# hassony2/handobjectconsist

Hardware: AMD Instinct MI355X
Metric: trainmeshwarp iters/sec (render+warp, B=64, 256x256) (higher is better)
Workload: dtype f32; 1 GPU; trainmeshwarp.py consist step, per-GPU B=64, 256x256, hand 778v/1552f + object 1002v/2000f (7104 faces after fill-back), ResNet-18 fp32 (MIOpen convolutions, channels-last, + fused HIP BatchNorm/ReLU/residual/max-pool kernels), Adam; global_batch=64, image_size=256, parallelism=dp1

## Files before the change

handobjectconsist_amd/_lib.py:

```python
import ctypes
import os

import torch

_HERE = os.path.dirname(os.path.abspath(__file__))
LIB_PATH = os.environ.get("HOC_LIB_PATH") or os.path.join(_HERE, "libmeshraster_hip.so")
ABI_VERSION = 9
FLAG_REFERENCE_ALGO = 1
FLAG_SPARSE_TILES = 2
FLAG_OUTPUT_ZEROED = 4
FLAG_TILE_PER_WORKGROUP = 8
FLAG_TILE_LIST_CLEARED = 16
FLAG_FORCE_PARTS = 1 << 24
FLAG_ONE_WORKGROUP_PER_IMAGE = 32 << 24
FLAG_PARTS_IN_ONE_LAUNCH = 64 << 24
FLAG_PLAIN_DIVISIONS = 4096 << 8
FLAG_FORCE_GATHER = 32 << 8
FLAG_COUNT_PIXEL_MAP_TERMS = 1024 << 8
CRITERION_L1 = 0
CRITERION_L2 = 1
DTYPE_F32, DTYPE_BF16, DTYPE_U8 = 0, 1, 2
DTYPE_CODES = {torch.float32: DTYPE_F32, torch.bfloat16: DTYPE_BF16, torch.uint8: DTYPE_U8}
IMAGE_DTYPES = (torch.float32, torch.bfloat16)
MASK_DTYPES = (torch.float32, torch.uint8)
# ... 88 lines not shown
    "mr_pair_step_forward": (_I, [_P, _P]),
    "mr_pair_step_backward": (_I, [_P, _P]),
    "mr_frames_to_batch_workspace_bytes": (_L, [_I, _I, _I]),
    "mr_frames_to_batch": (_I, [_P] * 3 + [_F] * 6 + [_P, _L, _P, _P] + [_I] * 6 + [_P]),
    "mr_frames_to_batch_typed": (_I, [_P] * 3 + [_F] * 6 + [_P, _L, _P, _P] + [_I] * 6 + [_P, _I, _I]),
    "mr_frames_color_augment_workspace_bytes": (_L, [_I, _I, _I]),
    "mr_frames_color_augment": (_I, [_P] * 7 + [_L, _I, _I, _I, _P]),
    "mr_jpeg_info": (_I, [_P, _L, _P]),
    "mr_jpeg_packed_bytes": (_L, [_I] * 5),
    "mr_jpeg_entropy_decode": (_I, [_P, _L, _P, _L]),
    "mr_jpeg_reconstruct_workspace_bytes": (_L, [_I] * 6),
    "mr_jpeg_reconstruct": (_I, [_P] + [_I] * 6 + [_P, _P, _L, _P]),
    "mr_png_packed_bytes": (_L, [_I] * 3),
    "mr_png_unfilter_workspace_bytes": (_L, [_I] * 4),
    "mr_png_unfilter": (_I, [_P] + [_I] * 4 + [_P, _P, _P]),
    "mr_frames_resize_taps": (_I, [_I, _I]),
    "mr_frames_resize_tables": (_I, [_I, _I, _P, _P]),
    "mr_frames_resize_plan": (_I, [_I] * 4 + [_P]),
    "mr_frames_resize_workspace_bytes": (_I, [_I] * 5),
    "mr_frames_resize": (_I, [_P, _I, _I, _I, _P, _I, _I] + [_P] * 6),
    "mr_bn_act_forward": (_I, [_P] * 6 + [_F, _I, _I, _I, _P, _I, _I, _I, _P]),
    "mr_bn_act_backward_workspace_bytes": (_L, [_I, _I]),
    "mr_bn_act_backward": (_I, [_P] * 8 + [_F, _I, _I, _I] + [_P] * 5 + [_L, _I, _I, _I, _P]),
    "mr_bn_add_bn_act_forward": (_I, [_P] * 6 + [_F] + [_P] * 4 + [_F, _I, _P, _I, _I, _I, _P]),
    "mr_bn_add_bn_act_backward_workspace_bytes": (_L, [_I, _I]),
    "mr_bn_add_bn_act_backward": (_I, [_P] * 8 + [_F] + [_P] * 4 + [_F, _I] + [_P] * 7 + [_L, _I, _I, _I, _P]),
    "mr_stem_pool_forward": (_I, [_P] * 5 + [_F, _I, _I, _P, _P, _I, _I, _I, _I, _P]),
    "mr_stem_pool_records_bytes": (_L, [_I, _I, _I, _I]),
    "mr_stem_pool_backward_workspace_bytes": (_L, [_I, _I, _I, _I]),
    "mr_stem_pool_backward": (_I, [_P] * 8 + [_F, _I, _I] + [_P] * 4 + [_L, _I, _I, _I, _I, _P]),
    "mr_stem_pool_param_grads": (_I, [_P] * 7 + [_F, _I] + [_P] * 3 + [_L, _I, _I, _I, _I, _P]),
    "mr_stem_conv_wrw_tiling": (_I, [_P] * 3),
    "mr_stem_conv_wrw_workspace_bytes": (_L, [_I, _I, _I, _I]),
    "mr_stem_conv_wrw": (_I, [_P] * 7 + [_F, _P, _P, _I, _P, _L] + [_I] * 8 + [_P]),
}

_lib = None


def load():
    global _lib
    if _lib is not None:
        return _lib
    if not os.path.exists(LIB_PATH):
        raise RuntimeError(
            f"{LIB_PATH} is missing: the HIP extension has not been built. Run "
# ... 95 lines not shown
```

handobjectconsist_amd/csrc/bn_device.hpp:

```cpp
#pragma once
#include <initializer_list>

#include "mr_common.hpp"

namespace mr {

__device__ __forceinline__ float act_to_f32(float v) { return v; }
__device__ __forceinline__ float act_to_f32(bf16_t v) { return bf16_to_f32(v); }
template <typename T> __device__ __forceinline__ T act_from_f32(float v);
template <> __device__ __forceinline__ float act_from_f32<float>(float v) { return v; }
template <> __device__ __forceinline__ bf16_t act_from_f32<bf16_t>(float v) { return f32_to_bf16(v); }

template <typename T> struct Vec4;
template <> struct Vec4<float> { typedef float4 type; };
template <> struct Vec4<bf16_t> { typedef ushort4 type; };

template <typename T>
__device__ __forceinline__ float load1(const void* base, int64_t o) { return act_to_f32(static_cast<const T*>(base)[o]); }
template <typename T>
__device__ __forceinline__ void store1(void* base, int64_t o, float v) { static_cast<T*>(base)[o] = act_from_f32<T>(v); }
template <typename T>
__device__ __forceinline__ void load4(const void* base, int64_t o, float* v) {
    const typename Vec4<T>::type t = *reinterpret_cast<const typename Vec4<T>::type*>(static_cast<const T*>(base) + o);
    v[0] = act_to_f32(t.x); v[1] = act_to_f32(t.y); v[2] = act_to_f32(t.z); v[3] = act_to_f32(t.w);
}
template <typename T>
__device__ __forceinline__ void store4(void* base, int64_t o, const float* v) {
    typename Vec4<T>::type t;
    t.x = act_from_f32<T>(v[0]); t.y = act_from_f32<T>(v[1]); t.z = act_from_f32<T>(v[2]); t.w = act_from_f32<T>(v[3]);
    *reinterpret_cast<typename Vec4<T>::type*>(static_cast<T*>(base) + o) = t;
}

template <typename T>
__device__ __forceinline__ float load1_grad(const void* grad_y, const void* grad_y2, int64_t o) {
    float g = load1<T>(grad_y, o);
    if (grad_y2) g += load1<T>(grad_y2, o);
    return g;
}
template <typename T>
__device__ __forceinline__ void load4_grad(const void* grad_y, const void* grad_y2, int64_t o, float* g) {
    load4<T>(grad_y, o, g);
    if (grad_y2) {
        float g2[4];
        load4<T>(grad_y2, o, g2);
#pragma unroll
        for (int i = 0; i < 4; i++) g[i] += g2[i];
    }
}

__device__ __forceinline__ float relu_nan(float z) { return z > 0.0f ? z : (z != z ? z : 0.0f); }

struct BnAffine {
    const float* weight;
// ... 144 lines not shown
```

handobjectconsist_amd/csrc/frozen_bn.hip:

```cpp
#include "bn_device.hpp"

namespace mr {

struct BnParams {
    const void* x;
    const void* residual;
    BnAffine bn;
    int relu;
    int N, C, HW, split;
    void* y;
    const void* grad_y;
    const void* grad_y2;
    void* grad_x;
    void* grad_residual;
    float* partial;
};

template <bool BACKWARD>
__device__ __forceinline__ void bn_act_element(float x, bool has_res, float res, float grad, bool relu, float mean, float a,
                                               float b, float& out, float& gres, float& sum_g, float& sum_gd) {
    const float d = x - mean;
    float z = d * a + b;
    if (has_res) z = z + res;
    if (!BACKWARD) {
        out = relu ? relu_nan(z) : z;
    } else {
        const float g = (relu && !(z > 0.0f)) ? 0.0f : grad;
        gres = g;
        out = g * a;
        sum_g += g;
        sum_gd += g * d;
    }
}

template <typename T, bool VEC, bool BACKWARD>
__global__ __launch_bounds__(256) void bn_act_kernel(BnParams p) {
    const int c = blockIdx.x / p.split, k = blockIdx.x % p.split;
    const int n0 = (int)((int64_t)k * p.N / p.split), n1 = (int)((int64_t)(k + 1) * p.N / p.split);
// ... 21 lines not shown
#pragma unroll
        for (int i = 0; i < W; i++) bn_act_element<BACKWARD>(xv[i], has_res, rv[i], gv[i], relu, mean, a, b, out[i], gres[i], s[0], s[1]);
        void* dst = BACKWARD ? p.grad_x : p.y;
        if (VEC) {
            store4<T>(dst, o, out);
            if (BACKWARD && p.grad_residual) store4<T>(p.grad_residual, o, gres);
        } else {
            store1<T>(dst, o, out[0]);
            if (BACKWARD && p.grad_residual) store1<T>(p.grad_residual, o, gres[0]);
        }
    }
    if (BACKWARD && p.partial) {
        float t[2];
        wave_block_sums<2>(s, t);
        if (threadIdx.x == 0) {
            p.partial[(int64_t)c * p.split + k] = t[0];
            p.partial[(int64_t)(p.C + c) * p.split + k] = t[1];
        }
    }
}

constexpr int BN_NHWC_BLOCKS = 2048;

template <typename T, bool BACKWARD>
__global__ __launch_bounds__(256) void bn_act_nhwc_kernel(BnParams p) {
    const NhwcLane l = nhwc_lane(p.bn, p.C);
    const int64_t pixels = (int64_t)p.N * p.HW;
    const bool relu = p.relu != 0, has_res = p.residual != nullptr;
    float s[2][4] = {};
    for (int64_t px = l.first(); px < pixels; px += l.stride()) {
        const int64_t o = px * p.C + l.c0;
        float xv[4], rv[4] = {}, gv[4] = {}, out[4], gres[4];
        load4<T>(p.x, o, xv);
        if (has_res) load4<T>(p.residual, o, rv);
        if (BACKWARD) load4_grad<T>(p.grad_y, p.grad_y2, o, gv);
#pragma unroll
        for (int i = 0; i < 4; i++)
            bn_act_element<BACKWARD>(xv[i], has_res, rv[i], gv[i], relu, l.mean[i], l.a[i], l.b[i], out[i], gres[i], s[0][i], s[1][i]);
        store4<T>(BACKWARD ? p.grad_x : p.y, o, out);
        if (BACKWARD && p.grad_residual) store4<T>(p.grad_residual, o, gres);
    }
    if (BACKWARD && p.partial) nhwc_block_sums<2>(l, s, p.partial, p.C);
}

struct BnAddParams {
    const void* x;
    const void* xd;
    BnAffine bn, bn_d;
    int N, C, HW;
    void* y;
    const void* grad_y;
    const void* grad_y2;
    void* grad_x;
    void* grad_xd;
    float* partial;
};

template <typename T, bool BACKWARD>
__global__ __launch_bounds__(256) void bn_add_bn_act_nhwc_kernel(BnAddParams p) {
    const NhwcLane l = nhwc_lane(p.bn, p.C), ld = nhwc_lane(p.bn_d, p.C);
    const int64_t pixels = (int64_t)p.N * p.HW;
    float s[3][4] = {};
    for (int64_t px = l.first(); px < pixels; px += l.stride()) {
// ... 102 lines not shown
    if (channels_last && channels > 0 && !nhwc_channels_ok(channels)) return MR_ERR_BADARG;
    if (channels == 0) return MR_OK;
    if (!weight || !bias || !running_mean || !running_var) return MR_ERR_BADARG;
    const bool want_params = grad_weight || grad_bias;
    if (batch_size == 0 || plane == 0) return zero_param_grads({grad_weight, grad_bias}, channels, (hipStream_t)stream);
    if (!grad_y || !x || !grad_x) return MR_ERR_BADARG;
    if (grad_residual && !residual) return MR_ERR_BADARG;
    if (want_params && (!workspace || workspace_bytes < mr_bn_act_backward_workspace_bytes(batch_size, channels)))
        return MR_ERR_BADARG;
    BnParams p = bn_fill(x, residual, weight, bias, running_mean, running_var, eps, relu, batch_size, channels, plane);
    p.grad_y = grad_y; p.grad_y2 = grad_y2; p.grad_x = grad_x; p.grad_residual = grad_residual;
    p.partial = want_params ? static_cast<float*>(workspace) : nullptr;
    if (!bn_sizes_ok(p)) return MR_ERR_BADARG;
    const bool all_aligned = aligned4(x, act_dtype) && aligned4(grad_y, act_dtype) && aligned4(grad_y2, act_dtype) &&
                             aligned4(grad_x, act_dtype) && aligned4(residual, act_dtype) && aligned4(grad_residual, act_dtype);
    if (channels_last && !all_aligned) return MR_ERR_BADARG;
    const int64_t slots = bn_act_slots(batch_size, channels, channels_last, (int64_t)batch_size * plane);
    bn_launch<true>(p, act_dtype, channels_last, plane % 4 == 0 && all_aligned, (int)slots, (hipStream_t)stream);
    MR_CHECK_LAUNCH();
    if (!want_params) return MR_OK;
    return launch_bn_finish<2>(p.partial, slots, channels, bn_finish_out(running_var, eps, grad_weight, grad_bias), (hipStream_t)stream);
}

namespace mr {
static BnAddParams bn_add_fill(const void* x, const void* xd, const BnAffine& bn, const BnAffine& bn_d, int N, int C, int plane) {
    BnAddParams p{};
    p.x = x; p.xd = xd; p.bn = bn; p.bn_d = bn_d; p.N = N; p.C = C; p.HW = plane;
    return p;
}
template <bool BACKWARD>
static void bn_add_launch(const BnAddParams& p, int act_dtype, int blocks, hipStream_t s) {
    dispatch_act(act_dtype, [&](auto tag) {
        using T = typename decltype(tag)::type;
        hipLaunchKernelGGL((bn_add_bn_act_nhwc_kernel<T, BACKWARD>), dim3((unsigned)blocks), dim3(256), 0, s, p);
    });
}
}

extern "C" int mr_bn_add_bn_act_forward(const void* x, const void* xd, const float* weight, const float* bias,
                                        const float* running_mean, const float* running_var, float eps,
                                        const float* weight_d, const float* bias_d, const float* running_mean_d,
                                        const float* running_var_d, float eps_d, int act_dtype, void* y, int batch_size,
                                        int channels, int plane, mr_stream_t stream) {
    using namespace mr;
    if (batch_size < 0 || channels < 0 || plane < 0 || (act_dtype != 0 && act_dtype != 1)) return MR_ERR_BADARG;
    if (channels > 0 && !nhwc_channels_ok(channels)) return MR_ERR_BADARG;
// ... 54 lines not shown
```

handobjectconsist_amd/csrc/stem_pool.hip:

```cpp
#include "bn_device.hpp"

namespace mr {

struct StemParams {
    const void* x;
    BnAffine bn;
    int N, C, H, W, OH, OW;
    int tiles_x, tiles_y;
    void* y;
    const void* grad_y;
    const void* grad_y2;
    void* grad_x;
    float* partial;
    unsigned char* argmax;
};

constexpr int SP_TX = 32, SP_TY = 16;
constexpr int SP_IH = 2 * SP_TY + 3, SP_IW = 2 * SP_TX + 8, SP_C0 = 4;
constexpr int SP_LDW = SP_IW + 1;

template <typename T, bool KEEP_D>
__device__ __forceinline__ void load_tile(const StemParams& p, const T* xp, int oy0, int ox0, float mean, float a,
                                          float b, float (*zt)[SP_LDW], float (*dt)[SP_LDW]) {
    const int iy0 = 2 * oy0 - 1, ix0 = 2 * ox0 - SP_C0;
// ... 199 lines not shown
                g[0] += id.x == code ? gv[0] : 0.0f;
                g[1] += id.y == code ? gv[1] : 0.0f;
                g[2] += id.z == code ? gv[2] : 0.0f;
                g[3] += id.w == code ? gv[3] : 0.0f;
            }
        }
#pragma unroll
        for (int i = 0; i < 4; i++) {
            const float d = xv[i] - l.mean[i];
            const float gm = (d * l.a[i] + l.b[i] > 0.0f) ? g[i] : 0.0f;
            out[i] = gm * l.a[i];
            s[0][i] += gm;
            s[1][i] += gm * d;
        }
        store4<T>(p.grad_x, ip * p.C + l.c0, out);
    }
    if (p.partial) nhwc_block_sums<2>(l, s, p.partial, p.C);
}

__device__ __forceinline__ unsigned char* sp_rec_codes(const StemParams& p) {
    return p.argmax + (int64_t)p.N * p.OH * p.OW * p.C * 4;
}

template <typename T>
__global__ __launch_bounds__(256) void stem_pool_rec_forward_kernel(StemParams p) {
    const NhwcLane l = nhwc_lane(p.bn, p.C);
    float* rec_d = reinterpret_cast<float*>(p.argmax);
    unsigned char* rec_code = sp_rec_codes(p);
    const int QH = (p.OH + 1) >> 1, QW = (p.OW + 1) >> 1;
    const int64_t total = (int64_t)p.N * QH * QW;
    for (int64_t q = l.first(); q < total; q += l.stride()) {
        const int qx = (int)(q % QW), qy = (int)((q / QW) % QH), n = (int)(q / ((int64_t)QW * QH));
        const int oy0 = 2 * qy, ox0 = 2 * qx;
        float best[2][2][4], bd[2][2][4];
        unsigned bi[2][2][4];
#pragma unroll
        for (int w = 0; w < 4; w++)
#pragma unroll
            for (int i = 0; i < 4; i++) { best[w >> 1][w & 1][i] = -__builtin_inff(); bd[w >> 1][w & 1][i] = 0.0f; bi[w >> 1][w & 1][i] = 0; }
#pragma unroll
        for (int r = 0; r < 5; r++) {
            const int iy = 2 * oy0 - 1 + r;
            if (iy < 0 || iy >= p.H) continue;
#pragma unroll
            for (int c = 0; c < 5; c++) {
                const int ix = 2 * ox0 - 1 + c;
                if (ix < 0 || ix >= p.W) continue;
                float xv[4];
                load4<T>(p.x, (((int64_t)n * p.H + iy) * p.W + ix) * p.C + l.c0, xv);
#pragma unroll
                for (int i = 0; i < 4; i++) {
                    const float d = xv[i] - l.mean[i];
                    const float v = relu_nan(d * l.a[i] + l.b[i]);
#pragma unroll
                    for (int wy = 0; wy < 2; wy++) {
                        const int kh = r - 2 * wy;
                        if (kh < 0 || kh > 2) continue;
#pragma unroll
                        for (int wx = 0; wx < 2; wx++) {
                            const int kw = c - 2 * wx;
                            if (kw < 0 || kw > 2) continue;
                            if (v > best[wy][wx][i] || v != v) { best[wy][wx][i] = v; bd[wy][wx][i] = d; bi[wy][wx][i] = (unsigned)(kh * 3 + kw); }
                        }
                    }
                }
            }
        }
#pragma unroll
        for (int wy = 0; wy < 2; wy++)
#pragma unroll
            for (int wx = 0; wx < 2; wx++) {
                const int oy = oy0 + wy, ox = ox0 + wx;
                if (oy >= p.OH || ox >= p.OW) continue;
                const int64_t o = (((int64_t)n * p.OH + oy) * p.OW + ox) * p.C + l.c0;
                store4<T>(p.y, o, best[wy][wx]);
                *reinterpret_cast<float4*>(rec_d + o) = make_float4(bd[wy][wx][0], bd[wy][wx][1], bd[wy][wx][2], bd[wy][wx][3]);
                *reinterpret_cast<uchar4*>(rec_code + o) = make_uchar4((unsigned char)bi[wy][wx][0], (unsigned char)bi[wy][wx][1],
                                                                       (unsigned char)bi[wy][wx][2], (unsigned char)bi[wy][wx][3]);
            }
    }
}

template <typename T>
__global__ __launch_bounds__(256) void stem_pool_rec_backward_kernel(StemParams p) {
    const NhwcLane l = nhwc_lane(p.bn, p.C);
    const float* rec_d = reinterpret_cast<const float*>(p.argmax);
    const unsigned char* rec_code = sp_rec_codes(p);
    const int QH = (p.H >> 1) + 1, QW = (p.W >> 1) + 1;
    const int64_t total = (int64_t)p.N * QH * QW;
    float sums[2][4] = {};
// ... 237 lines not shown
```

handobjectconsist_amd/csrc/stem_wrw.hip:

```cpp
#include "bn_device.hpp"

namespace mr {

constexpr int SW_TY = 4, SW_TX = 32;
constexpr int SW_BLOCKS = 512;
constexpr int SW_C = 64;
constexpr int SW_TAPS = 7 * 7 * 3;
constexpr int SW_NB = 5;
constexpr int SW_OUT = SW_C * SW_TAPS;
constexpr int SW_PH = 2 * SW_TY + 5;
constexpr int SW_PROW = (2 * SW_TX + 5) * 3;
constexpr int SW_PW = 213;
constexpr int SW_G = SW_TY * SW_TX * SW_C;
constexpr int SW_LDS = SW_G + SW_PH * SW_PW;
constexpr int SW_FIN_RUNS = 8, SW_FIN_RUN = SW_BLOCKS / SW_FIN_RUNS;
static_assert(SW_LDS >= SW_C * SW_NB * 32, "the wave reduction reuses the tile's LDS");
static_assert(SW_OUT % 32 == 0, "finish kernel: 32 outputs per workgroup");

typedef float f32x16 __attribute__((ext_vector_type(16)));

struct WrwParams {
    const float* grad_y;
    const float* grad_y2;
    const float* rec_d;
    const unsigned char* rec_code;
    BnAffine bn;
    const float* image;
    float* partial;
    int N, Hin, Win, H, W, OH, OW;
    int tiles_x, tiles_y;
    int64_t tiles;
};

__device__ __forceinline__ void wrw_keep(float& v) { asm volatile("" : "+v"(v)); }
__device__ __forceinline__ void wrw_keep(unsigned& v) { asm volatile("" : "+v"(v)); }
__device__ __forceinline__ void wrw_keep(float4& v) { asm volatile("" : "+v"(v.x), "+v"(v.y), "+v"(v.z), "+v"(v.w)); }

__global__ __launch_bounds__(256, 2) void stem_conv_wrw_kernel(WrwParams p) {
    __shared__ __attribute__((aligned(16))) float lds[SW_LDS];
    float* const G = lds;
    float* const patch = lds + SW_G;
    const int tid = threadIdx.x, lane = tid & 63, wave = tid >> 6, half = lane >> 5, l31 = lane & 31;

    const int c0 = 4 * (tid & 15), qcol = tid >> 4;
    float a[4], b[4];
#pragma unroll
    for (int i = 0; i < 4; i++) {
        float mean;
        channel_consts(p.bn, c0 + i, mean, a[i], b[i]);
    }

    const float* aptr[2];
    const float* bptr[SW_NB];
#pragma unroll
    for (int m = 0; m < 2; m++) aptr[m] = G + (wave * SW_TX + 16 * half) * SW_C + ((l31 + 32 * m) ^ (32 * half));
#pragma unroll
    for (int n = 0; n < SW_NB; n++) {
        const int t = l31 + 32 * n;
        const int off = t < SW_TAPS ? (t / 21) * SW_PW + t % 21 : 0;
        bptr[n] = patch + 2 * wave * SW_PW + 6 * 16 * half + off;
// ... 4 lines not shown
    for (int m = 0; m < 2; m++)
#pragma unroll
        for (int n = 0; n < SW_NB; n++)
#pragma unroll
            for (int r = 0; r < 16; r++) acc[m][n][r] = 0.0f;

    const int per_image = p.tiles_x * p.tiles_y;
    for (int64_t tile = blockIdx.x; tile < p.tiles; tile += gridDim.x) {
        const int n = (int)(tile / per_image), rem = (int)(tile - (int64_t)n * per_image);
        const int cy0 = (rem / p.tiles_x) * SW_TY, cx0 = (rem % p.tiles_x) * SW_TX;

        {
            const int iy0 = 2 * cy0 - 3, ix0 = 2 * cx0 - 3;
            const int c = tid < SW_PROW ? tid : SW_PROW - 1, ix = ix0 + c / 3;
            const bool col = ix >= 0 && ix < p.Win;
            const float* src = p.image + (int64_t)n * p.Hin * p.Win * 3 + (col ? ix0 * 3 + c : 0);
            float pv[SW_PH];
#pragma unroll
            for (int r = 0; r < SW_PH; r++) {
                const int iy = iy0 + r, iyc = iy < 0 ? 0 : (iy >= p.Hin ? p.Hin - 1 : iy);
                pv[r] = src[(int64_t)iyc * p.Win * 3];
            }
#pragma unroll
            for (int r = 0; r < SW_PH; r++) wrw_keep(pv[r]);
#pragma unroll
            for (int r = 0; r < SW_PH; r++) {
                const int iy = iy0 + r;
                if (!col || iy < 0 || iy >= p.Hin) pv[r] = 0.0f;
            }
            if (tid < SW_PROW) {
#pragma unroll
                for (int r = 0; r < SW_PH; r++) patch[r * SW_PW + tid] = pv[r];
            }
        }

#pragma unroll 1
        for (int qr = 0; qr < SW_TY / 2; qr++) {
            float s[2][2][4];
            unsigned code[2][2][4];
            unsigned idw[2][2];
            float4 dv[2][2], g1[2][2], g2[2][2];
#pragma unroll
            for (int j = 0; j < 2; j++)
#pragma unroll
                for (int k = 0; k < 2; k++) {
                    const int wy = (cy0 >> 1) + qr + j, wx = (cx0 >> 1) + qcol + k;
                    const int64_t o = (((int64_t)n * p.OH + (wy < p.OH ? wy : p.OH - 1)) * p.OW + (wx < p.OW ? wx : p.OW - 1)) * SW_C + c0;
                    idw[j][k] = *reinterpret_cast<const unsigned*>(p.rec_code + o);
                    dv[j][k] = *reinterpret_cast<const float4*>(p.rec_d + o);
                    g1[j][k] = *reinterpret_cast<const float4*>(p.grad_y + o);
                    g2[j][k] = *reinterpret_cast<const float4*>((p.grad_y2 ? p.grad_y2 : p.grad_y) + o);
                }
#pragma unroll
            for (int j = 0; j < 2; j++)
#pragma unroll
                for (int k = 0; k < 2; k++) { wrw_keep(idw[j][k]); wrw_keep(dv[j][k]); wrw_keep(g1[j][k]); wrw_keep(g2[j][k]); }
#pragma unroll
            for (int j = 0; j < 2; j++)
#pragma unroll
                for (int k = 0; k < 2; k++) {
                    const int wy = (cy0 >> 1) + qr + j, wx = (cx0 >> 1) + qcol + k;
                    const bool win = wy < p.OH && wx < p.OW;
                    const float d[4] = {dv[j][k].x, dv[j][k].y, dv[j][k].z, dv[j][k].w};
                    const float gv[4] = {p.grad_y2 ? g1[j][k].x + g2[j][k].x : g1[j][k].x, p.grad_y2 ? g1[j][k].y + g2[j][k].y : g1[j][k].y,
                                         p.grad_y2 ? g1[j][k].z + g2[j][k].z : g1[j][k].z, p.grad_y2 ? g1[j][k].w + g2[j][k].w : g1[j][k].w};
#pragma unroll
                    for (int i = 0; i < 4; i++) {
                        code[j][k][i] = win ? (idw[j][k] >> (8 * i)) & 255u : 255u;
                        s[j][k][i] = (d[i] * a[i] + b[i] > 0.0f) ? gv[i] : 0.0f;
                    }
                }
#pragma unroll
            for (int pr = 0; pr < 2; pr++)
#pragma unroll
                for (int pc = 0; pc < 2; pc++) {
                    const int py = 2 * qr + pr, px = 2 * qcol + pc;
                    float g[4] = {0.0f, 0.0f, 0.0f, 0.0f};
#pragma unroll
                    for (int dy = 0; dy < 2; dy++) {
// ... 135 lines not shown
```

handobjectconsist_amd/models/synthnet.py:

```python
import os

import numpy as np
import torch
import torch.nn.functional as F
from torch import nn

from handobjectconsist_amd import _lib
from handobjectconsist_amd.models import manoadapt
from handobjectconsist_amd.nn import frozen_bn
from handobjectconsist_amd.utils import project as camproject
from handobjectconsist_amd.utils import synth


USE_HIP_BN = os.environ.get("HOC_HIP_BN", "1") == "1"


USE_CHANNELS_LAST = os.environ.get("HOC_CHANNELS_LAST", "1") == "1"


USE_STEM_WRW = True


def _fused_bn(bn, x):
    if not (USE_HIP_BN and not bn.training and x.is_cuda):
        return False
    out_dtype = torch.get_autocast_dtype("cuda") if torch.is_autocast_enabled("cuda") else x.dtype
    return out_dtype in (torch.float32, torch.bfloat16)


class BasicBlock(nn.Module):
    expansion = 1

    def __init__(self, inplanes, planes, stride=1, downsample=None):
        super().__init__()
        self.conv1 = nn.Conv2d(inplanes, planes, 3, stride, 1, bias=False)
        self.bn1 = nn.BatchNorm2d(planes)
        self.relu = nn.ReLU(inplace=True)
        self.conv2 = nn.Conv2d(planes, planes, 3, 1, 1, bias=False)
        self.bn2 = nn.BatchNorm2d(planes)
        self.downsample = downsample

    def forward_fused(self, x, x_identity, dup=False):
        if self.downsample is not None:
            xd = self.downsample[0](x_identity)
            out = frozen_bn.bn_act(self.conv1(x), self.bn1)
            return frozen_bn.bn_add_bn_act(self.conv2(out), self.bn2, xd, self.downsample[1], dup=dup)
        out = frozen_bn.bn_act(self.conv1(x), self.bn1)
        return frozen_bn.bn_act(self.conv2(out), self.bn2, residual=x_identity, dup=dup)

    def forward(self, x):
        if _fused_bn(self.bn1, x):
            return self.forward_fused(x, x)
        residual = x if self.downsample is None else self.downsample(x)
        out = self.relu(self.bn1(self.conv1(x)))
        out = self.bn2(self.conv2(out))
        return self.relu(out + residual)


class ResNet18Features(nn.Module):

    def __init__(self):
        super().__init__()
        self.inplanes = 64
        self.conv1 = nn.Conv2d(3, 64, kernel_size=7, stride=2, padding=3, bias=False)
        self.bn1 = nn.BatchNorm2d(64)
        self.relu = nn.ReLU(inplace=True)
        self.maxpool = nn.MaxPool2d(kernel_size=3, stride=2, padding=1)
        self.layer1 = self._make_layer(64, 2)
        self.layer2 = self._make_layer(128, 2, stride=2)
        self.layer3 = self._make_layer(256, 2, stride=2)
        self.layer4 = self._make_layer(512, 2, stride=2)
# ... 486 lines not shown
```

handobjectconsist_amd/nn/frozen_bn.py:

```python
import torch
import torch.nn.functional as F

from handobjectconsist_amd import _lib


_ACT_DTYPES = {torch.float32: 0, torch.bfloat16: 1}


def _nhwc_channels_ok(C):
    return 4 <= C <= 1024 and 1024 % C == 0


def _layout(x):
    if (x.dim() == 4 and _nhwc_channels_ok(x.shape[1]) and not x.is_contiguous()
            and x.is_contiguous(memory_format=torch.channels_last)):
        return x, 1
    return x.contiguous(), 0


def _aligned(t, cl):
    if t is not None and cl and t.data_ptr() % (4 * t.element_size()):
        return t.clone(memory_format=torch.preserve_format)
    return t

# ... 47 lines not shown
        return (y, y.view_as(y)) if dup else y

    @staticmethod
    def backward(ctx, grad_y, grad_y2=None):
        xc, rc, w, b, m, v = ctx.saved_tensors
        eps, relu, N, C, plane, cl = ctx.cfg
        need_x, need_r, need_w, need_b = ctx.needs_input_grad[:4]
        g, g2 = _incoming(grad_y, grad_y2, xc.dtype, cl)
        if g is None:
            return (None,) * 9
        dev = xc.device
        grad_x = torch.empty_like(xc)
        grad_r = torch.empty_like(xc) if (rc is not None and need_r) else None
        grad_w = torch.empty_like(w) if need_w else None
        grad_b = torch.empty_like(b) if need_b else None
        work, wbytes = _workspace("mr_bn_act_backward_workspace_bytes", (N, C), dev, need_w or need_b)
        _lib.call("mr_bn_act_backward", _lib.ptr(g), _lib.ptr(g2), _lib.ptr(xc), _lib.ptr(rc), _lib.ptr(w), _lib.ptr(b), _lib.ptr(m),
                  _lib.ptr(v), eps, int(relu), _ACT_DTYPES[xc.dtype], cl, _lib.ptr(grad_x), _lib.ptr(grad_r), _lib.ptr(grad_w),
                  _lib.ptr(grad_b),
                  _lib.ptr(work), wbytes, N, C, plane, _lib.stream_ptr(dev))
        return (grad_x if need_x else None), grad_r, grad_w, grad_b, None, None, None, None, None


def bn_act(x, bn, residual=None, relu=True, dup=False):
    if bn.training or not bn.track_running_stats:
        raise RuntimeError("bn_act needs frozen BatchNorm statistics (module.eval())")
    return _BnActFunction.apply(x, residual, bn.weight, bn.bias, bn.running_mean, bn.running_var, bn.eps, relu, dup)


class _BnAddBnActFunction(torch.autograd.Function):

    @staticmethod
    def forward(ctx, x, xd, weight, bias, running_mean, running_var, eps, weight_d, bias_d, running_mean_d,
                running_var_d, eps_d, dup):
        ctx.set_materialize_grads(False)
        _lib.check_cuda(x, xd, weight, bias, running_mean, running_var, weight_d, bias_d, running_mean_d, running_var_d)
        xc, xdc = _aligned(x, 1), _aligned(xd, 1)
        N, C = xc.shape[:2]
        plane = xc[0, 0].numel() if N and C else 0
        chan = _channel_arrays(C, weight, bias, running_mean, running_var, weight_d, bias_d, running_mean_d, running_var_d)
        y = torch.empty_like(xc)
        _lib.call("mr_bn_add_bn_act_forward", _lib.ptr(xc), _lib.ptr(xdc), *[_lib.ptr(t) for t in chan[:4]], float(eps),
                  *[_lib.ptr(t) for t in chan[4:]], float(eps_d), _ACT_DTYPES[xc.dtype], _lib.ptr(y), N, C, plane,
                  _lib.stream_ptr(xc.device))
        ctx.save_for_backward(xc, xdc, *chan)
        ctx.cfg = (float(eps), float(eps_d), N, C, plane)
        return (y, y.view_as(y)) if dup else y

    @staticmethod
# ... 153 lines not shown
```

include/meshraster_hip.h:

```cpp
#ifndef MESHRASTER_HIP_H
#define MESHRASTER_HIP_H

#include <stdint.h>

#ifdef __cplusplus
extern "C" {
#endif

#define MR_OK 0
#define MR_ERR_BADARG (-1)
#define MR_ERR_NOTIMPL (-2)

#define MR_FLAG_REFERENCE_ALGO 1
#define MR_FLAG_SPARSE_TILES 2
#define MR_FLAG_OUTPUT_ZEROED 4
#define MR_FLAG_TILE_PER_WORKGROUP 8
#define MR_FLAG_TILE_LIST_CLEARED 16
#define MR_FLAG_FORCE_PARTS (1 << 24)
#define MR_FLAG_ONE_WORKGROUP_PER_IMAGE (32 << 24)
#define MR_FLAG_PARTS_IN_ONE_LAUNCH (64 << 24)
#define MR_FLAG_PLAIN_DIVISIONS (4096 << 8)
#define MR_FLAG_FORCE_GATHER (32 << 8)
#define MR_FLAG_COUNT_PIXEL_MAP_TERMS (1024 << 8)

// ... 532 lines not shown
#define MR_RESIZE_MAX_TAPS 33
#define MR_RESIZE_PLAN_INTS 8
MR_API int mr_frames_resize_taps(int in_size, int out_size);
MR_API int mr_frames_resize_tables(int in_size, int out_size, int* bounds, int* coeffs);
MR_API int mr_frames_resize_plan(int src_w, int src_h, int dst_w, int dst_h, int* plan);
MR_API int mr_frames_resize_workspace_bytes(int num_frames, int src_w, int src_h, int dst_w, int dst_h);
MR_API int mr_frames_resize(const unsigned char* frames_in, int num_frames, int src_w, int src_h,
                            unsigned char* frames_out, int dst_w, int dst_h, const int* bounds_x, const int* coeffs_x,
                            const int* bounds_y, const int* coeffs_y, void* workspace, mr_stream_t stream);

MR_API int mr_bn_act_forward(const void* x, const void* residual, const float* weight, const float* bias,
                             const float* running_mean, const float* running_var, float eps, int relu,
                             int act_dtype, int channels_last, void* y, int batch_size, int channels,
                             int plane, mr_stream_t stream);
MR_API int64_t mr_bn_act_backward_workspace_bytes(int batch_size, int channels);
MR_API int mr_bn_act_backward(const void* grad_y, const void* grad_y2, const void* x, const void* residual,
                              const float* weight, const float* bias, const float* running_mean,
                              const float* running_var, float eps, int relu, int act_dtype,
                              int channels_last, void* grad_x, void* grad_residual, float* grad_weight,
                              float* grad_bias,
                              void* workspace, int64_t workspace_bytes, int batch_size, int channels,
                              int plane, mr_stream_t stream);

MR_API int mr_bn_add_bn_act_forward(const void* x, const void* xd, const float* weight, const float* bias,
                                    const float* running_mean, const float* running_var, float eps,
                                    const float* weight_d, const float* bias_d, const float* running_mean_d,
                                    const float* running_var_d, float eps_d, int act_dtype, void* y,
                                    int batch_size, int channels, int plane, mr_stream_t stream);
MR_API int64_t mr_bn_add_bn_act_backward_workspace_bytes(int batch_size, int channels);
MR_API int mr_bn_add_bn_act_backward(const void* grad_y, const void* grad_y2, const void* x, const void* xd,
                                     const float* weight, const float* bias, const float* running_mean,
                                     const float* running_var, float eps, const float* weight_d,
                                     const float* bias_d, const float* running_mean_d, const float* running_var_d,
                                     float eps_d, int act_dtype, void* grad_x, void* grad_xd, float* grad_weight,
                                     float* grad_bias, float* grad_weight_d, float* grad_bias_d, void* workspace,
                                     int64_t workspace_bytes, int batch_size, int channels, int plane,
                                     mr_stream_t stream);

MR_API int mr_stem_pool_forward(const void* x, const float* weight, const float* bias,
                                const float* running_mean, const float* running_var, float eps,
                                int act_dtype, int channels_last, void* y, unsigned char* argmax,
                                int batch_size, int channels, int height, int width, mr_stream_t stream);
MR_API int64_t mr_stem_pool_records_bytes(int batch_size, int channels, int height, int width);
MR_API int64_t mr_stem_pool_backward_workspace_bytes(int batch_size, int channels, int height, int width);
MR_API int mr_stem_pool_backward(const void* grad_y, const void* grad_y2, const void* x,
                                 const unsigned char* argmax,
// ... 26 lines not shown
```

Before: 39.08 iters/s (one optimiser step = 1 data batch + 1 consist batch of B per GPU; roofline.stock_trunk_it_s = the same step with the trunk's BatchNorm/ReLU/max-pool on the stock nn modules).

## Save ReLU sign bitmask in residual BN+ReLU to skip residual reload in backward

Adds a forward/backward variant of the fused BN+residual+ReLU kernel that packs the ReLU output signs into a per-wave ballot bitmask. Backward then reads one bit per element instead of re-reading the residual tensor, and the residual no longer has to be kept alive for autograd. This cuts backward memory traffic and saved-activation memory, at the cost of extra ballot work and bitmask writes in the forward pass. Separately, the stem pool forward loads each row's five taps up front, with clamped indices and an asm barrier, to raise memory-level parallelism.

```diff
diff --git a/handobjectconsist_amd/_lib.py b/handobjectconsist_amd/_lib.py
--- a/handobjectconsist_amd/_lib.py
+++ b/handobjectconsist_amd/_lib.py
@@ -134,6 +134,8 @@
     "mr_bn_act_forward": (_I, [_P] * 6 + [_F, _I, _I, _I, _P, _I, _I, _I, _P]),
     "mr_bn_act_backward_workspace_bytes": (_L, [_I, _I]),
     "mr_bn_act_backward": (_I, [_P] * 8 + [_F, _I, _I, _I] + [_P] * 5 + [_L, _I, _I, _I, _P]),
+    "mr_bn_act_signs_forward": (_I, [_P] * 6 + [_F, _I, _P, _P, _L, _I, _I, _I, _P]),
+    "mr_bn_act_signs_backward": (_I, [_P] * 4 + [_L] + [_P] * 4 + [_F, _I] + [_P] * 5 + [_L, _I, _I, _I, _P]),
     "mr_bn_add_bn_act_forward": (_I, [_P] * 6 + [_F] + [_P] * 4 + [_F, _I, _P, _I, _I, _I, _P]),
     "mr_bn_add_bn_act_backward_workspace_bytes": (_L, [_I, _I]),
     "mr_bn_add_bn_act_backward": (_I, [_P] * 8 + [_F] + [_P] * 4 + [_F, _I] + [_P] * 7 + [_L, _I, _I, _I, _P]),
diff --git a/handobjectconsist_amd/csrc/bn_device.hpp b/handobjectconsist_amd/csrc/bn_device.hpp
--- a/handobjectconsist_amd/csrc/bn_device.hpp
+++ b/handobjectconsist_amd/csrc/bn_device.hpp
@@ -29,6 +29,23 @@
     typename Vec4<T>::type t;
     t.x = act_from_f32<T>(v[0]); t.y = act_from_f32<T>(v[1]); t.z = act_from_f32<T>(v[2]); t.w = act_from_f32<T>(v[3]);
     *reinterpret_cast<typename Vec4<T>::type*>(static_cast<T*>(base) + o) = t;
+}
+
+template <typename T>
+__device__ __forceinline__ typename Vec4<T>::type load4_raw(const void* base, int64_t o) {
+    return *reinterpret_cast<const typename Vec4<T>::type*>(static_cast<const T*>(base) + o);
+}
+template <typename V>
+__device__ __forceinline__ void widen4(const V& t, float* v) {
+    v[0] = act_to_f32(t.x); v[1] = act_to_f32(t.y); v[2] = act_to_f32(t.z); v[3] = act_to_f32(t.w);
+}
+
+__device__ __forceinline__ void keep_loaded(float& v) { asm volatile("" : "+v"(v)); }
+__device__ __forceinline__ void keep_loaded(unsigned& v) { asm volatile("" : "+v"(v)); }
+__device__ __forceinline__ void keep_loaded(float4& v) { asm volatile("" : "+v"(v.x), "+v"(v.y), "+v"(v.z), "+v"(v.w)); }
+__device__ __forceinline__ void keep_loaded(ushort4& v) {
+    uint2& u = reinterpret_cast<uint2&>(v);
+    asm volatile("" : "+v"(u.x), "+v"(u.y));
 }
 
 template <typename T>
diff --git a/handobjectconsist_amd/csrc/frozen_bn.hip b/handobjectconsist_amd/csrc/frozen_bn.hip
--- a/handobjectconsist_amd/csrc/frozen_bn.hip
+++ b/handobjectconsist_amd/csrc/frozen_bn.hip
@@ -14,6 +14,7 @@
     void* grad_x;
     void* grad_residual;
     float* partial;
+    unsigned long long* signs;
 };
 
 template <bool BACKWARD>
@@ -81,23 +82,80 @@
 
 constexpr int BN_NHWC_BLOCKS = 2048;
 
+static inline int64_t bn_signs_bytes(int N, int C, int plane) { return ((int64_t)N * plane * C + 255) / 256 * 32; }
+
+template <typename T>
+__device__ __forceinline__ void bn_signs_forward_walk(const BnParams& p, const NhwcLane& l, int64_t pixels) {
+    const unsigned lane = threadIdx.x & 63;
+    for (int64_t px = l.first();; px += l.stride()) {
+        const bool active = px < pixels;
+        if (__ballot(active) == 0) break;
+        const int64_t o = px * p.C + l.c0;
+        float xv[4] = {}, rv[4] = {}, out[4], gres, s0 = 0.0f, s1 = 0.0f;
+        if (active) {
+            load4<T>(p.x, o, xv);
+            load4<T>(p.residual, o, rv);
+        }
+        unsigned long long word = 0;
+#pragma unroll
+        for (int i = 0; i < 4; i++) {
+            bn_act_element<false>(xv[i], true, rv[i], 0.0f, true, l.mean[i], l.a[i], l.b[i], out[i], gres, s0, s1);
+            const unsigned long long w = __ballot(active && out[i] > 0.0f);
+            if (lane == (unsigned)i) word = w;
+        }
+        if (active) store4<T>(p.y, o, out);
+        if (lane < 4) p.signs[(o >> 8) * 4 + lane] = word;
+    }
+}
+
+template <typename T>
+__device__ __forceinline__ void bn_signs_backward_walk(const BnParams& p, const NhwcLane& l, int64_t pixels, float (&s)[2][4]) {
+    const unsigned lane = threadIdx.x & 63;
+    for (int64_t px = l.first(); px < pixels; px += l.stride()) {
+        const int64_t o = px * p.C + l.c0;
+        const int64_t seg = o >> 8;
+        const unsigned seg_lo = __builtin_amdgcn_readfirstlane((unsigned)seg), seg_hi = __builtin_amdgcn_readfirstlane((unsigned)(seg >> 32));
+        const unsigned long long* words = p.signs + 4 * (((unsigned long long)seg_hi << 32) | seg_lo);
+        const unsigned long long w[4] = {words[0], words[1], words[2], words[3]};
+        float xv[4], gv[4], out[4], gres[4];
+        load4<T>(p.x, o, xv);
+        load4_grad<T>(p.grad_y, p.grad_y2, o, gv);
+#pragma unroll
+        for (int i = 0; i < 4; i++) {
+            const float d = xv[i] - l.mean[i];
+            const float g = ((w[i] >> lane) & 1ull) ? gv[i] : 0.0f;
+            gres[i] = g;
+            out[i] = g * l.a[i];
+            s[0][i] += g;
+            s[1][i] += g * d;
+        }
+        store4<T>(p.grad_x, o, out);
+        if (p.grad_residual) store4<T>(p.grad_residual, o, gres);
+    }
+}
+
 template <typename T, bool BACKWARD>
 __global__ __launch_bounds__(256) void bn_act_nhwc_kernel(BnParams p) {
     const NhwcLane l = nhwc_lane(p.bn, p.C);
     const int64_t pixels = (int64_t)p.N * p.HW;
     const bool relu = p.relu != 0, has_res = p.residual != nullptr;
     float s[2][4] = {};
-    for (int64_t px = l.first(); px < pixels; px += l.stride()) {
-        const int64_t o = px * p.C + l.c0;
-        float xv[4], rv[4] = {}, gv[4] = {}, out[4], gres[4];
-        load4<T>(p.x, o, xv);
-        if (has_res) load4<T>(p.residual, o, rv);
-        if (BACKWARD) load4_grad<T>(p.grad_y, p.grad_y2, o, gv);
+    if (p.signs) {
+        if (BACKWARD) bn_signs_backward_walk<T>(p, l, pixels, s);
+        else bn_signs_forward_walk<T>(p, l, pixels);
+    } else {
+        for (int64_t px = l.first(); px < pixels; px += l.stride()) {
+            const int64_t o = px * p.C + l.c0;
+            float xv[4], rv[4] = {}, gv[4] = {}, out[4], gres[4];
+            load4<T>(p.x, o, xv);
+            if (has_res) load4<T>(p.residual, o, rv);
+            if (BACKWARD) load4_grad<T>(p.grad_y, p.grad_y2, o, gv);
 #pragma unroll
-        for (int i = 0; i < 4; i++)
-            bn_act_element<BACKWARD>(xv[i], has_res, rv[i], gv[i], relu, l.mean[i], l.a[i], l.b[i], out[i], gres[i], s[0][i], s[1][i]);
-        store4<T>(BACKWARD ? p.grad_x : p.y, o, out);
-        if (BACKWARD && p.grad_residual) store4<T>(p.grad_residual, o, gres);
+            for (int i = 0; i < 4; i++)
+                bn_act_element<BACKWARD>(xv[i], has_res, rv[i], gv[i], relu, l.mean[i], l.a[i], l.b[i], out[i], gres[i], s[0][i], s[1][i]);
+            store4<T>(BACKWARD ? p.grad_x : p.y, o, out);
+            if (BACKWARD && p.grad_residual) store4<T>(p.grad_residual, o, gres);
+        }
     }
     if (BACKWARD && p.partial) nhwc_block_sums<2>(l, s, p.partial, p.C);
 }
@@ -246,6 +304,57 @@
     return launch_bn_finish<2>(p.partial, slots, channels, bn_finish_out(running_var, eps, grad_weight, grad_bias), (hipStream_t)stream);
 }
 
+extern "C" int mr_bn_act_signs_forward(const void* x, const void* residual, const float* weight, const float* bias,
+                                       const float* running_mean, const float* running_var, float eps, int act_dtype, void* y,
+                                       void* signs, int64_t signs_bytes, int batch_size, int channels, int plane,
+                                       mr_stream_t stream) {
+    using namespace mr;
+    if (batch_size < 0 || channels < 0 || plane < 0 || (act_dtype != 0 && act_dtype != 1)) return MR_ERR_BADARG;
+    if (channels > 0 && !nhwc_channels_ok(channels)) return MR_ERR_BADARG;
+    if (signs_bytes < bn_signs_bytes(batch_size, channels, plane)) return MR_ERR_BADARG;
+    if (batch_size == 0 || channels == 0 || plane == 0) return MR_OK;
+    if (!x || !residual || !weight || !bias || !running_mean || !running_var || !y || !signs) return MR_ERR_BADARG;
+    BnParams p = bn_fill(x, residual, weight, bias, running_mean, running_var, eps, 1, batch_size, channels, plane);
+    p.y = y;
+    p.signs = static_cast<unsigned long long*>(signs);
+    if (!bn_sizes_ok(p)) return MR_ERR_BADARG;
+    if (!aligned4(x, act_dtype) || !aligned4(y, act_dtype) || !aligned4(residual, act_dtype) || misaligned({signs}, 7)) return MR_ERR_BADARG;
+    bn_launch<false>(p, act_dtype, 1, true, nhwc_blocks((int64_t)batch_size * plane, channels, BN_NHWC_BLOCKS), (hipStream_t)stream);
+    MR_CHECK_LAUNCH();
+    return MR_OK;
+}
+
+extern "C" int mr_bn_act_signs_backward(const void* grad_y, const void* grad_y2, const void* x, const void* signs,
+                                        int64_t signs_bytes, const float* weight, const float* bias, const float* running_mean,
+                                        const float* running_var, float eps, int act_dtype, void* grad_x, void* grad_residual,
+                                        float* grad_weight, float* grad_bias, void* workspace, int64_t workspace_bytes,
+                                        int batch_size, int channels, int plane, mr_stream_t stream) {
+    using namespace mr;
+    if (batch_size < 0 || channels < 0 || plane < 0 || (act_dtype != 0 && act_dtype != 1)) return MR_ERR_BADARG;
+    if (channels > 0 && !nhwc_channels_ok(channels)) return MR_ERR_BADARG;
+    if (signs_bytes < bn_signs_bytes(batch_size, channels, plane)) return MR_ERR_BADARG;
+    if (channels == 0) return MR_OK;
+    if (!weight || !bias || !running_mean || !running_var) return MR_ERR_BADARG;
+    const bool want_params = grad_weight || grad_bias;
+    if (batch_size == 0 || plane == 0) return zero_param_grads({grad_weight, grad_bias}, channels, (hipStream_t)stream);
+    if (!grad_y || !x || !signs || !grad_x) return MR_ERR_BADARG;
+    if (want_params && (!workspace || workspace_bytes < mr_bn_act_backward_workspace_bytes(batch_size, channels)))
+        return MR_ERR_BADARG;
+    BnParams p = bn_fill(x, nullptr, weight, bias, running_mean, running_var, eps, 1, batch_size, channels, plane);
+    p.grad_y = grad_y; p.grad_y2 = grad_y2; p.grad_x = grad_x; p.grad_residual = grad_residual;
+    p.partial = want_params ? static_cast<float*>(workspace) : nullptr;
+    p.signs = const_cast<unsigned long long*>(static_cast<const unsigned long long*>(signs));
+    if (!bn_sizes_ok(p)) return MR_ERR_BADARG;
+    if (!aligned4(x, act_dtype) || !aligned4(grad_y, act_dtype) || !aligned4(grad_y2, act_dtype) || !aligned4(grad_x, act_dtype) ||
+        !aligned4(grad_residual, act_dtype) || misaligned({signs}, 7))
+        return MR_ERR_BADARG;
+    const int64_t slots = bn_act_slots(batch_size, channels, 1, (int64_t)batch_size * plane);
+    bn_launch<true>(p, act_dtype, 1, true, (int)slots, (hipStream_t)stream);
+    MR_CHECK_LAUNCH();
+    if (!want_params) return MR_OK;
+    return launch_bn_finish<2>(p.partial, slots, channels, bn_finish_out(running_var, eps, grad_weight, grad_bias), (hipStream_t)stream);
+}
+
 namespace mr {
 static BnAddParams bn_add_fill(const void* x, const void* xd, const BnAffine& bn, const BnAffine& bn_d, int N, int C, int plane) {
     BnAddParams p{};
diff --git a/handobjectconsist_amd/csrc/stem_pool.hip b/handobjectconsist_amd/csrc/stem_pool.hip
--- a/handobjectconsist_amd/csrc/stem_pool.hip
+++ b/handobjectconsist_amd/csrc/stem_pool.hip
@@ -245,6 +245,43 @@
     return p.argmax + (int64_t)p.N * p.OH * p.OW * p.C * 4;
 }
 
+template <typename T, int R>
+__device__ __forceinline__ void sp_rec_row(const StemParams& p, const NhwcLane& l, int n, int oy0, int ox0, float (&best)[2][2][4],
+                                           float (&bd)[2][2][4], unsigned (&bi)[2][2][4]) {
+    typename Vec4<T>::type raw[5];
+    const int iy = 2 * oy0 - 1 + R, iyc = iy < 0 ? 0 : (iy >= p.H ? p.H - 1 : iy);
+#pragma unroll
+    for (int c = 0; c < 5; c++) {
+        const int ix = 2 * ox0 - 1 + c, ixc = ix < 0 ? 0 : (ix >= p.W ? p.W - 1 : ix);
+        raw[c] = load4_raw<T>(p.x, (((int64_t)n * p.H + iyc) * p.W + ixc) * p.C + l.c0);
+    }
+#pragma unroll
+    for (int c = 0; c < 5; c++) keep_loaded(raw[c]);
+#pragma unroll
+    for (int c = 0; c < 5; c++) {
+        const int ix = 2 * ox0 - 1 + c;
+        const bool in = iy >= 0 && iy < p.H && ix >= 0 && ix < p.W;
+        float xv[4];
+        widen4(raw[c], xv);
+#pragma unroll
+        for (int i = 0; i < 4; i++) {
+            const float d = xv[i] - l.mean[i];
+            const float v = relu_nan(d * l.a[i] + l.b[i]);
+#pragma unroll
+            for (int wy = 0; wy < 2; wy++) {
+                const int kh = R - 2 * wy;
+                if (kh < 0 || kh > 2) continue;
+#pragma unroll
+                for (int wx = 0; wx < 2; wx++) {
+                    const int kw = c - 2 * wx;
+                    if (kw < 0 || kw > 2) continue;
+                    if (in && (v > best[wy][wx][i] || v != v)) { best[wy][wx][i] = v; bd[wy][wx][i] = d; bi[wy][wx][i] = (unsigned)(kh * 3 + kw); }
+                }
+            }
+        }
+    }
+}
+
 template <typename T>
 __global__ __launch_bounds__(256) void stem_pool_rec_forward_kernel(StemParams p) {
     const NhwcLane l = nhwc_lane(p.bn, p.C);
@@ -261,34 +298,11 @@
         for (int w = 0; w < 4; w++)
 #pragma unroll
             for (int i = 0; i < 4; i++) { best[w >> 1][w & 1][i] = -__builtin_inff(); bd[w >> 1][w & 1][i] = 0.0f; bi[w >> 1][w & 1][i] = 0; }
-#pragma unroll
-        for (int r = 0; r < 5; r++) {
-            const int iy = 2 * oy0 - 1 + r;
-            if (iy < 0 || iy >= p.H) continue;
-#pragma unroll
-            for (int c = 0; c < 5; c++) {
-                const int ix = 2 * ox0 - 1 + c;
-                if (ix < 0 || ix >= p.W) continue;
-                float xv[4];
-                load4<T>(p.x, (((int64_t)n * p.H + iy) * p.W + ix) * p.C + l.c0, xv);
-#pragma unroll
-                for (int i = 0; i < 4; i++) {
-                    const float d = xv[i] - l.mean[i];
-                    const float v = relu_nan(d * l.a[i] + l.b[i]);
-#pragma unroll
-                    for (int wy = 0; wy < 2; wy++) {
-                        const int kh = r - 2 * wy;
-                        if (kh < 0 || kh > 2) continue;
-#pragma unroll
-                        for (int wx = 0; wx < 2; wx++) {
-                            const int kw = c - 2 * wx;
-                            if (kw < 0 || kw > 2) continue;
-                            if (v > best[wy][wx][i] || v != v) { best[wy][wx][i] = v; bd[wy][wx][i] = d; bi[wy][wx][i] = (unsigned)(kh * 3 + kw); }
-                        }
-                    }
-                }
-            }
-        }
+        sp_rec_row<T, 0>(p, l, n, oy0, ox0, best, bd, bi);
+        sp_rec_row<T, 1>(p, l, n, oy0, ox0, best, bd, bi);
+        sp_rec_row<T, 2>(p, l, n, oy0, ox0, best, bd, bi);
+        sp_rec_row<T, 3>(p, l, n, oy0, ox0, best, bd, bi);
+        sp_rec_row<T, 4>(p, l, n, oy0, ox0, best, bd, bi);
 #pragma unroll
         for (int wy = 0; wy < 2; wy++)
 #pragma unroll
diff --git a/handobjectconsist_amd/csrc/stem_wrw.hip b/handobjectconsist_amd/csrc/stem_wrw.hip
--- a/handobjectconsist_amd/csrc/stem_wrw.hip
+++ b/handobjectconsist_amd/csrc/stem_wrw.hip
@@ -32,10 +32,6 @@
     int64_t tiles;
 };
 
-__device__ __forceinline__ void wrw_keep(float& v) { asm volatile("" : "+v"(v)); }
-__device__ __forceinline__ void wrw_keep(unsigned& v) { asm volatile("" : "+v"(v)); }
-__device__ __forceinline__ void wrw_keep(float4& v) { asm volatile("" : "+v"(v.x), "+v"(v.y), "+v"(v.z), "+v"(v.w)); }
-
 __global__ __launch_bounds__(256, 2) void stem_conv_wrw_kernel(WrwParams p) {
     __shared__ __attribute__((aligned(16))) float lds[SW_LDS];
     float* const G = lds;
@@ -86,7 +82,7 @@
                 pv[r] = src[(int64_t)iyc * p.Win * 3];
             }
 #pragma unroll
-            for (int r = 0; r < SW_PH; r++) wrw_keep(pv[r]);
+            for (int r = 0; r < SW_PH; r++) keep_loaded(pv[r]);
 #pragma unroll
             for (int r = 0; r < SW_PH; r++) {
                 const int iy = iy0 + r;
@@ -118,7 +114,7 @@
 #pragma unroll
             for (int j = 0; j < 2; j++)
 #pragma unroll
-                for (int k = 0; k < 2; k++) { wrw_keep(idw[j][k]); wrw_keep(dv[j][k]); wrw_keep(g1[j][k]); wrw_keep(g2[j][k]); }
+                for (int k = 0; k < 2; k++) { keep_loaded(idw[j][k]); keep_loaded(dv[j][k]); keep_loaded(g1[j][k]); keep_loaded(g2[j][k]); }
 #pragma unroll
             for (int j = 0; j < 2; j++)
 #pragma unroll
diff --git a/handobjectconsist_amd/models/synthnet.py b/handobjectconsist_amd/models/synthnet.py
--- a/handobjectconsist_amd/models/synthnet.py
+++ b/handobjectconsist_amd/models/synthnet.py
@@ -46,7 +46,7 @@
             out = frozen_bn.bn_act(self.conv1(x), self.bn1)
             return frozen_bn.bn_add_bn_act(self.conv2(out), self.bn2, xd, self.downsample[1], dup=dup)
         out = frozen_bn.bn_act(self.conv1(x), self.bn1)
-        return frozen_bn.bn_act(self.conv2(out), self.bn2, residual=x_identity, dup=dup)
+        return frozen_bn.bn_act(self.conv2(out), self.bn2, residual=x_identity, dup=dup, signs=True)
 
     def forward(self, x):
         if _fused_bn(self.bn1, x):
diff --git a/handobjectconsist_amd/nn/frozen_bn.py b/handobjectconsist_amd/nn/frozen_bn.py
--- a/handobjectconsist_amd/nn/frozen_bn.py
+++ b/handobjectconsist_amd/nn/frozen_bn.py
@@ -93,9 +93,65 @@
         return (grad_x if need_x else None), grad_r, grad_w, grad_b, None, None, None, None, None
 
 
-def bn_act(x, bn, residual=None, relu=True, dup=False):
+def signs_bytes(numel):
+    return (numel + 255) // 256 * 32
+
+
+class _BnActSignsFunction(torch.autograd.Function):
+
+    @staticmethod
+    def forward(ctx, x, residual, weight, bias, running_mean, running_var, eps, dup):
+        ctx.set_materialize_grads(False)
+        _lib.check_cuda(x, residual, weight, bias, running_mean, running_var)
+        if residual.shape != x.shape or residual.dtype != x.dtype:
+            raise ValueError("residual must match x")
+        xc = _aligned(x, 1)
+        rc = _aligned(residual.contiguous(memory_format=torch.channels_last), 1)
+        N, C = xc.shape[:2]
+        plane = xc[0, 0].numel() if N and C else 0
+        w, b, m, v = _channel_arrays(C, weight, bias, running_mean, running_var)
+        y = torch.empty_like(xc)
+        sbytes = signs_bytes(xc.numel())
+        signs = torch.empty((sbytes,), dtype=torch.uint8, device=xc.device)
+        _lib.call("mr_bn_act_signs_forward", _lib.ptr(xc), _lib.ptr(rc), _lib.ptr(w), _lib.ptr(b), _lib.ptr(m), _lib.ptr(v),
+                  float(eps), _ACT_DTYPES[xc.dtype], _lib.ptr(y), _lib.ptr(signs), sbytes, N, C, plane,
+                  _lib.stream_ptr(xc.device))
+        ctx.save_for_backward(xc, signs, w, b, m, v)
+        ctx.cfg = (float(eps), N, C, plane)
+        return (y, y.view_as(y)) if dup else y
+
+    @staticmethod
+    def backward(ctx, grad_y, grad_y2=None):
+        xc, signs, w, b, m, v = ctx.saved_tensors
+        eps, N, C, plane = ctx.cfg
+        need_x, need_r, need_w, need_b = ctx.needs_input_grad[:4]
+        g, g2 = _incoming(grad_y, grad_y2, xc.dtype, 1)
+        if g is None:
+            return (None,) * 8
+        dev = xc.device
+        grad_x = torch.empty_like(xc)
+        grad_r = torch.empty_like(xc) if need_r else None
+        grad_w = torch.empty_like(w) if need_w else None
+        grad_b = torch.empty_like(b) if need_b else None
+        work, wbytes = _workspace("mr_bn_act_backward_workspace_bytes", (N, C), dev, need_w or need_b)
+        _lib.call("mr_bn_act_signs_backward", _lib.ptr(g), _lib.ptr(g2), _lib.ptr(xc), _lib.ptr(signs), signs.numel(),
+                  _lib.ptr(w), _lib.ptr(b), _lib.ptr(m), _lib.ptr(v), eps, _ACT_DTYPES[xc.dtype], _lib.ptr(grad_x),
+                  _lib.ptr(grad_r), _lib.ptr(grad_w), _lib.ptr(grad_b), _lib.ptr(work), wbytes, N, C, plane,
+                  _lib.stream_ptr(dev))
+        return (grad_x if need_x else None), grad_r, grad_w, grad_b, None, None, None, None
+
+
+def _signs_apply(x, residual, relu):
+    return (residual is not None and relu and x.is_cuda and x.dtype in _ACT_DTYPES and x.dim() == 4 and x.numel() > 0
+            and residual.shape == x.shape and residual.dtype == x.dtype
+            and _nhwc_channels_ok(x.shape[1]) and not x.is_contiguous() and x.is_contiguous(memory_format=torch.channels_last))
+
+
+def bn_act(x, bn, residual=None, relu=True, dup=False, signs=False):
     if bn.training or not bn.track_running_stats:
         raise RuntimeError("bn_act needs frozen BatchNorm statistics (module.eval())")
+    if signs and _signs_apply(x, residual, relu):
+        return _BnActSignsFunction.apply(x, residual, bn.weight, bn.bias, bn.running_mean, bn.running_var, bn.eps, dup)
     return _BnActFunction.apply(x, residual, bn.weight, bn.bias, bn.running_mean, bn.running_var, bn.eps, relu, dup)
 
 
diff --git a/include/meshraster_hip.h b/include/meshraster_hip.h
--- a/include/meshraster_hip.h
+++ b/include/meshraster_hip.h
@@ -578,6 +578,17 @@
                               void* workspace, int64_t workspace_bytes, int batch_size, int channels,
                               int plane, mr_stream_t stream);
 
+MR_API int mr_bn_act_signs_forward(const void* x, const void* residual, const float* weight, const float* bias,
+                                   const float* running_mean, const float* running_var, float eps, int act_dtype,
+                                   void* y, void* signs, int64_t signs_bytes, int batch_size, int channels, int plane,
+                                   mr_stream_t stream);
+MR_API int mr_bn_act_signs_backward(const void* grad_y, const void* grad_y2, const void* x, const void* signs,
+                                    int64_t signs_bytes, const float* weight, const float* bias,
+                                    const float* running_mean, const float* running_var, float eps, int act_dtype,
+                                    void* grad_x, void* grad_residual, float* grad_weight, float* grad_bias,
+                                    void* workspace, int64_t workspace_bytes, int batch_size, int channels, int plane,
+                                    mr_stream_t stream);
+
 MR_API int mr_bn_add_bn_act_forward(const void* x, const void* xd, const float* weight, const float* bias,
                                     const float* running_mean, const float* running_var, float eps,
                                     const float* weight_d, const float* bias_d, const float* running_mean_d,
```

Result: no change. 39.21 iters/s (one optimiser step = 1 data batch + 1 consist batch of B per GPU; roofline.stock_trunk_it_s = the same step with the trunk's BatchNorm/ReLU/max-pool on the stock nn modules), median of 6 (+0.3%).
